# 2235854410/CCVPE

Measured on AMD Instinct MI355X. Metric: query images/sec (VIGOR, 512x512 sat / 320x640 grd), higher is better.
Workload: dtype f32; 1 GPU; vigor_samearea_fov360_b32; variant=vigor_ori_prior, batch_per_gpu=32, global_batch=32, parallelism=image-parallel x1, all_gather of 20 B/query results, schedule=two streams per GPU (aerial encoder + orientation decoder on the second)

## Files before the change

ccvpe_amd/csrc/ccvpe_api.hip:

```cpp
#include "ccvpe_internal.h"

namespace ccvpe { thread_local unsigned long long g_launches = 0; }
static thread_local std::string g_err_storage;
std::string& ccvpe_err() { return g_err_storage; }
int ccvpe_fail(int code, const char* fmt, ...) {
    char buf[1024];
    va_list ap;
    va_start(ap, fmt);
    vsnprintf(buf, sizeof(buf), fmt, ap);
    va_end(ap);
    g_err_storage = buf;
    return code;
}

__global__ __launch_bounds__(256) void checksum_kernel(const uint32_t* __restrict__ p, size_t n, unsigned long long* out) {
    unsigned long long s = 0;
    for (size_t i = (size_t)blockIdx.x * 256 + threadIdx.x; i < n; i += (size_t)gridDim.x * 256) s += (unsigned long long)p[i] * (unsigned long long)((i & 1023) + 1);
    for (int o = 32; o > 0; o >>= 1) s += __shfl_down(s, o);
    if ((threadIdx.x & 63) == 0) atomicAdd(out, s);
}


Switches read_switches() {
    Switches s;
    auto set = [](const char* name) { return getenv(name) != nullptr; };
    auto off = [](const char* name) { const char* e = getenv(name); return e && std::atoi(e) == 0; };
    if (const char* e = getenv("CCVPE_AUTOTUNE")) s.autotune = std::atoi(e) != 0;
    if (const char* e = getenv("CCVPE_FUSE_MBCONV")) s.fuse_mbconv = std::atoi(e);
    if (const char* e = getenv("CCVPE_FUSE_L1")) s.fuse_level1 = std::atoi(e) != 0;
    if (const char* e = getenv("CCVPE_L1_TILE")) s.l1_tile = std::atoi(e);
    if (const char* e = getenv("CCVPE_COMPOSE_L6")) s.compose_l6 = std::atoi(e);
    if (const char* e = getenv("CCVPE_WINOGRAD")) s.wino = std::atoi(e) != 0;
    if (const char* e = getenv("CCVPE_GRAPH")) s.graph_mode = std::atoi(e) != 0;
    if (const char* e = getenv("CCVPE_STREAMS")) s.two_streams = std::atoi(e) >= 2;
    if (const char* e = getenv("CCVPE_PRECISION")) s.precision = (std::string(e) == "bf16x3") ? 1 : 0;
    s.stem_dw = !off("CCVPE_STEM_DW");
    if (const char* e = getenv("CCVPE_FRONT_SPREAD")) s.front_spread = std::atoi(e);
    s.mbconv_image = !off("CCVPE_MBCONV_IMAGE");
    s.se_ticket = !off("CCVPE_SE_TICKET");
    if (const char* e = getenv("CCVPE_SE_PROLOGUE")) s.se_prologue = std::atoi(e) == 1;
    s.split_planes = !set("CCVPE_NO_SPLIT_PLANES");
    s.match_prep_early = !off("CCVPE_MATCH_PREP_EARLY");
    s.match_wide = !off("CCVPE_MATCH_WIDE");
    s.issue_interleaved = !off("CCVPE_ISSUE_ORDER");
    s.log_schedule = set("CCVPE_LOG_SCHEDULE");
    s.no_reuse = set("CCVPE_NO_REUSE");
// ... 290 lines not shown
            std::string nm = op.name;
            double issued = op.flops;
            if (const ConvTile* t = conv_tile(tile)) {
                nm += std::string("|") + t->name;
                if ((tile >> 8) == 255) nm += "_tailsplit";
                else if ((tile >> 8) > SPLIT_FUSED) nm += "_splitk" + std::to_string((tile >> 8) - SPLIT_FUSED) + "r";
                else if ((tile >> 8) > 1) nm += "_splitk" + std::to_string(tile >> 8);
                ConvParams q{};
                q.M = op.gemm_m; q.N = op.gemm_n;
                const double util = conv_tile_util(q, *t);
                const double mn_pad = util > 0 ? (double)op.gemm_m * op.gemm_n / util : 0.0;
                if (t->wino_f == 4) issued = 2.0 * mn_pad * 2.25 * ((op.conv_cin + 3) / 4 * 4);
                else if (t->wino_f == 2) issued = 2.0 * mn_pad * 4.0 * op.conv_cin;
                else issued = 2.0 * mn_pad * op.gemm_kpad * (t->family == TILE_BF16X3 ? 3.0 : 1.0);
            }
            h->prof.push_back({nm, ms, op.flops, op.bytes, issued});
        }
        (void)hipEventDestroy(e0);
        (void)hipEventDestroy(e1);
    }
    return 0;
}

static int run_forward(ccvpe_handle h, const ForwardCall& fc) {
    const PlanKey key = fc.plan_key();
    const int batch = fc.batch;
    if (!h || !fc.grd || (!fc.sat && !fc.cache) || (!fc.out && !key.pose)) return ccvpe_fail(CCVPE_EINVAL, "null argument");
    if (fc.cache && !fc.tile_index && batch > h->cfg.micro_batch) return ccvpe_fail(CCVPE_EINVAL, "cached forward needs batch <= micro_batch (%d)", h->cfg.micro_batch);
    if (fc.tile_index && fc.n_tiles > h->cfg.micro_batch)
        return ccvpe_fail(CCVPE_EINVAL, "n_tiles %d exceeds micro_batch (%d), the most ccvpe_encode_aerial writes", fc.n_tiles, h->cfg.micro_batch);
// ... 1096 lines not shown
```

ccvpe_amd/csrc/ccvpe_internal.h:

```cpp
#pragma once
#include "../../include/ccvpe.h"
#include "kernels.h"

#include <algorithm>
#include <cmath>
#include <cstdarg>
#include <cstdio>
#include <cstdlib>
#include <cstring>
#include <functional>
#include <map>
#include <memory>
#include <optional>
#include <set>
#include <string>
#include <type_traits>
#include <vector>

using namespace ccvpe;

std::string& ccvpe_err();
int ccvpe_fail(int code, const char* fmt, ...);
#define HIPCHK(expr)                                                                           \
    do {                                                                                       \
// ... 63 lines not shown
    int lo, hi; static_pad(k, s, lo, hi);
    return (n + lo + hi - k) / s + 1;
}
static int se_squeeze(int cin) { return std::max(1, (int)(cin * 0.25)); }
static int round_up(int a, int b) { return (a + b - 1) / b * b; }
static int deconv_width(const DecLevel& l, bool pad) {
    return (pad && l.skip > 0 && (l.dout * 4) % 64 != 0) ? round_up(l.dout, 16) : l.dout;
}

struct Switches {
    bool autotune = true;
    int fuse_mbconv = 1;
    bool fuse_level1 = true;
    int l1_tile = 1;
    std::optional<int> compose_l6;
    bool wino = true;
    int graph_mode = 0;
    bool two_streams = true;
    std::optional<int> precision;
    bool stem_dw = true;
    std::optional<int> front_spread;
    bool mbconv_image = true;
    bool se_ticket = true;
    bool se_prologue = false;
    bool split_planes = true;
    bool match_prep_early = true;
    bool match_wide = true;
    bool issue_interleaved = true;
    bool log_schedule = false;
    bool no_reuse = false;
// ... 60 lines not shown
    PackedConv head;
};
struct DecoderW {
    PackedConv deconv[6], conva[6], convb[5];
    float* tail_w = nullptr;
    float* l1_wt = nullptr;
    float tail_b[2] = {0.f, 0.f};
    float *l1_wc = nullptr, *l1_ws = nullptr, *l1_bc = nullptr;
    int l1_cx = 0, l1_cxp = 0, l1_c0 = 0, l1_ng = 0, l1_score = 0;
};
struct Level6W {
    float* wc = nullptr;
    float* bc = nullptr;
    PackedConv skip;
    int K = 0, Kc = 0, N = 0, Npad = 0;
};
static constexpr int LEVEL6_AUTO_MIN_BATCH = 8;
struct ccvpe_handle_s;
struct DecoderW;
int level6_shape(const ccvpe_handle_s* h, const DecoderW& d, const struct DecLevel& l, int& K, int& Kc, int& N, int& Npad);
int ensure_level6(ccvpe_handle_s* h, int wm);
void release_level6(ccvpe_handle_s* h);
int compose_level1(ccvpe_handle_s* h, DecoderW& d, const std::vector<float>& w, const std::vector<float>& b, const std::vector<float>& wa,
                   const std::vector<float>& ba, int cin, int nscore);
int pack_level1_tail(ccvpe_handle_s* h, DecoderW& d, const std::vector<float>& w2, const std::vector<float>& b2, int cout);

struct Tensor {
    int id = -1; int B = 0, H = 0, W = 0, C = 0;
    bool split = false;
    long long numel() const { return (long long)B * H * W * C; }
};

// ... 112 lines not shown

struct Op {
    std::string name;
    std::function<void(const Ctx&)> fn;
    std::vector<int> uses;
    double flops = 0, bytes = 0;
    std::shared_ptr<int> tile;
    int gemm_m = 0, gemm_n = 0, gemm_kpad = 0;
    int conv_cin = 0;
    bool bf16x3_only = false;
    bool wino_ok = false;
    bool wino4_ok = false;
    bool wino4x_ok = false;
    bool is_pw = false;
    bool proj_ok = false;
    int stream = 0;
    std::vector<int> wait_on;
    bool signal = false;
};

struct TapInfo { Tensor t; int coff; int C; };

struct Plan {
    PlanKey key;
    bool debug = false;
    std::vector<size_t> size;
    std::vector<size_t> off;
    std::vector<Op> ops;
    std::map<std::string, TapInfo> taps;
    size_t total = 0;
// ... 212 lines not shown
```

ccvpe_amd/csrc/ccvpe_plan.hip:

```cpp
#include "ccvpe_internal.h"

static int window_offset(const VariantSpec& vs, int level, int L) {
    const int C = vs.match_ch[level];
    return vs.centre ? (int)((double)C / 2 - (double)L / 2) : 0;
}
static int mod(int a, int m) { int r = a % m; return r < 0 ? r + m : r; }

ConvParams conv_params(const PackedConv& pc, const float* in, int in_ld, int B, int H, int W, int OH, int OW,
                              int stride, int pad_t, int pad_l, int act) {
    ConvParams p{};
    p.in = in; p.in_ld = in_ld; p.B = B; p.H = H; p.W = W; p.Cin = pc.cinp; p.OH = OH; p.OW = OW;
    p.KH = pc.KH; p.KW = pc.KW; p.stride = stride; p.pad_t = pad_t; p.pad_l = pad_l;
    p.wpk = pc.w; p.w_hi = pc.w_hi; p.w_lo = pc.w_lo; p.Kpad = pc.Kpad; p.Npad = round_up(pc.N, conv_igemm_npad()); p.nchunks = pc.nchunks; p.bias = pc.bias; p.N = pc.N; p.act = act;
    p.gate = nullptr; p.resid = nullptr; p.resid_ld = 0; p.ndst = 0; p.mode = MODE_CONV; p.deconv_cout = 0;
    p.M = B * OH * OW;
    p.in_bytes = (unsigned)((size_t)B * H * W * in_ld * sizeof(float));
    p.gate_bytes = (unsigned)((size_t)B * pc.cinp * sizeof(float));
    p.w_plane_bytes = (unsigned)((size_t)p.Npad * pc.Kpad * sizeof(unsigned short));
    p.wino_w = pc.wino; p.wino_n16 = pc.wino_n16; p.wino_bytes = (unsigned)pc.wino_bytes;
    p.wino4_w = pc.wino4; p.wino4_bytes = (unsigned)pc.wino4_bytes;
    p.wino4x_w = pc.wino4x; p.wino4x_bytes = (unsigned)pc.wino4x_bytes; p.wino4x_cfg = pc.wino4x_cfg;
    p.proj_w = pc.proj; p.proj_bytes = (unsigned)pc.proj_bytes;
    return p;
}
// ... 339 lines not shown
                : (B >= LEVEL6_AUTO_MIN_BATCH && !h->l6_failed) ? 4 : 0;
    Level6Params l6p[2] = {};
    if (l6_wm) {
        bool ok = true;
        for (int d = 0; d < 2; ++d) {
            Level6Params& q = l6p[d];
            q.wm = l6_wm; q.B = B;
            ok = ok && level6_shape(h, d ? h->ori : h->loc, d ? vs.ori[0] : vs.loc[0], q.K, q.Kc, q.N, q.Npad) == 0;
            q.R = level6_rows(B, l6_wm, &q.bm);
            ok = ok && level6_supported(q) && q.K == (d ? rpad + D : loc_in[0].C);
        }
        if (!ok && l6_forced) return ccvpe_fail(CCVPE_ESTATE, "composed level 6: the packed weights do not fit the plan's level-6 inputs");
        if (!ok) l6_wm = 0;
    }
    pl.l6_wm = l6_wm;
    Tensor skip15;
    ori_in6 = pl.alloc(B, 8, 8, rpad + D);
    pl.taps["ori_in6"] = {ori_in6, 0, ori_in6.C};

    EncOut genc, senc;
    if (!grd_cached) plan_encoder(h, pl, h->grd_enc, true, B, gh, gw, h->cfg.circular_padding != 0, nullptr, genc, "grd");
    TapDst td[5];
    for (int t = 0; t < 5; ++t) {
        td[t].n = 2;
        td[t].t[0] = loc_cat[t]; td[t].coff[0] = deconv_width(vs.loc[t], h->sw.pad_concat);
        td[t].t[1] = ori_cat[t]; td[t].coff[1] = deconv_width(vs.ori[t], h->sw.pad_concat);
    }
    if (l6_wm) td[0].n = 0;
    size_t coff[6];
    cache_layout(vs, B, coff);
// ... 68 lines not shown

    auto plan_level = [&](const DecoderW& dw, const DecLevel* lv, int j, Tensor din, Tensor cat, const std::string& tag) -> Tensor {
        const int hin = 8 << j, hout = hin * 2;
        const DecLevel& l = lv[j];
        Tensor mid = pl.alloc(B, hout, hout, l.mid);
        if (j == 0 && l6_wm) {
            const Level6W* w6 = &h->l6[&dw == &h->ori ? 1 : 0];
            const Level6Params lp = l6p[&dw == &h->ori ? 1 : 0];
            const int G = 4 * level6_positions(l6_wm);
            Tensor V = pl.alloc(G, 1, lp.R, lp.Kc), Mp = pl.alloc(G, 1, lp.R, lp.N), sk = pl.alloc(B, hout, hout, l.mid);
            const Tensor s15 = skip15;
            pl.add(tag + ".l6_transform", {din, V}, [=](const Ctx& c) {
                Level6Params q = lp; q.x = c.ptr(din); q.v = c.ptr(V);
                launch_level6_transform(q, c.stream);
            }, 0.0, 4.0 * ((double)din.numel() + (double)V.numel()));
            pl.add(tag + ".l6_gemm", {V, Mp}, [=](const Ctx& c) {
                Level6Params q = lp; q.v = c.ptr(V); q.wc = w6->wc; q.mp = c.ptr(Mp);
                launch_level6_gemm(q, c.stream);
            }, 2.0 * G * lp.R * (double)lp.N * lp.Kc, 4.0 * ((double)V.numel() + (double)G * lp.Npad * lp.Kc + (double)Mp.numel()));
            {
                const PackedConv* pc = &w6->skip;
                pl.add_conv(tag + ".conv_skip", {s15, sk}, B * hout * hout, lp.N, round_up(9 * l.skip, 32), [=](const Ctx& c, int tile) {
                    ConvParams p = conv_params(*pc, c.ptr(s15), s15.C, B, hout, hout, hout, hout, 1, 1, 1, ACT_NONE);
                    p.dst[0] = c.dst(sk); p.ndst = 1;
                    c.launch_conv(p, tile);
                }, 2.0 * B * hout * hout * 9.0 * s15.C * l.mid, 4.0 * B * hout * hout * ((double)s15.C + l.mid));
                pl.ops.back().conv_cin = s15.C;
                pl.ops.back().wino_ok = l.skip % 8 == 0;
                pl.ops.back().wino4_ok = pl.ops.back().wino_ok && lp.N >= h->sw.wino4_min_n && !h->sw.no_wino4;
                pl.ops.back().wino4x_ok = pl.ops.back().wino_ok && lp.N >= 24 && conv_wino4x_config(lp.N) >= 0 && !h->sw.no_wino4x;
            }
            pl.add(tag + ".l6_combine", {Mp, sk, mid}, [=](const Ctx& c) {
                Level6Params q = lp; q.mp = c.ptr(Mp); q.skip = c.ptr(sk); q.bc = w6->bc; q.out = c.ptr(mid);
                launch_level6_combine(q, c.stream);
            }, 0.0, 4.0 * ((double)Mp.numel() + 2.0 * (double)mid.numel()));
// ... 16 lines not shown
                pl.add_conv(tag + ".conv_a", {cat, mid}, B * hout * hout, pc->N, pc->Kpad, [=](const Ctx& c, int tile) {
                    ConvParams p = conv_params(*pc, c.ptr(cat), cat.C, B, hout, hout, hout, hout, 1, 1, 1, ACT_RELU);
                    p.in_split = cat.split; p.in_plane_bytes = (unsigned)(cat.numel() * 2);
                    p.dst[0] = c.dst(mid); p.ndst = 1;
                    c.launch_conv(p, tile);
                }, 2.0 * B * hout * hout * 9.0 * cat.C * l.mid, 4.0 * B * hout * hout * ((double)cat.C + l.mid));
                pl.ops.back().bf16x3_only = cat.split;
                pl.ops.back().conv_cin = cat.C;
                pl.ops.back().wino_ok = pc->wino != nullptr && !cat.split && h->sw.wino && h->cfg.reserved[0] == 0;
                pl.ops.back().wino4_ok = pl.ops.back().wino_ok && pc->wino4 != nullptr;
                pl.ops.back().wino4x_ok = pl.ops.back().wino_ok && pc->wino4x != nullptr;
            }
        }
        if (j == 5) return mid;
        Tensor o = pl.alloc(B, hout, hout, l.out);
        {
            const PackedConv* pc = &dw.convb[j];
            pl.add_conv(tag + ".conv_b", {mid, o}, B * hout * hout, pc->N, pc->Kpad, [=](const Ctx& c, int tile) {
                ConvParams p = conv_params(*pc, c.ptr(mid), mid.C, B, hout, hout, hout, hout, 1, 1, 1, ACT_NONE);
                p.in_split = mid.split; p.in_plane_bytes = (unsigned)(mid.numel() * 2);
                p.dst[0] = {c.ptr(o), o.C, 0}; p.ndst = 1;
                c.launch_conv(p, tile);
            }, 2.0 * B * hout * hout * 9.0 * l.mid * l.out, 4.0 * B * hout * hout * ((double)l.mid + l.out));
            pl.ops.back().bf16x3_only = mid.split;
            pl.ops.back().conv_cin = mid.C;
            pl.ops.back().wino_ok = pc->wino != nullptr && !mid.split && h->sw.wino && h->cfg.reserved[0] == 0;
            pl.ops.back().wino4_ok = pl.ops.back().wino_ok && pc->wino4 != nullptr;
            pl.ops.back().wino4x_ok = pl.ops.back().wino_ok && pc->wino4x != nullptr;
        }
        return o;
    };
// ... 323 lines not shown
```

ccvpe_amd/csrc/ccvpe_weights.hip:

```cpp
#include "ccvpe_internal.h"

#include <unistd.h>

static void add_bn(std::map<std::string, std::vector<int64_t>>& m, const std::string& p, int c) {
    m[p + ".weight"] = {c}; m[p + ".bias"] = {c}; m[p + ".running_mean"] = {c}; m[p + ".running_var"] = {c};
    m[p + ".num_batches_tracked"] = {};
}
static void add_encoder(std::map<std::string, std::vector<int64_t>>& m, const std::string& p) {
    m[p + "._conv_stem.weight"] = {32, 3, 3, 3};
    add_bn(m, p + "._bn0", 32);
    for (int i = 0; i < 16; ++i) {
        const BlockSpec& b = B0[i];
        std::string q = p + "._blocks." + std::to_string(i);
        int mid = b.cin * b.e;
        if (b.e != 1) { m[q + "._expand_conv.weight"] = {mid, b.cin, 1, 1}; add_bn(m, q + "._bn0", mid); }
        m[q + "._depthwise_conv.weight"] = {mid, 1, b.k, b.k};
        add_bn(m, q + "._bn1", mid);
        int sq = se_squeeze(b.cin);
        m[q + "._se_reduce.weight"] = {sq, mid, 1, 1}; m[q + "._se_reduce.bias"] = {sq};
        m[q + "._se_expand.weight"] = {mid, sq, 1, 1}; m[q + "._se_expand.bias"] = {mid};
        m[q + "._project_conv.weight"] = {b.cout, mid, 1, 1};
        add_bn(m, q + "._bn2", b.cout);
    }
    m[p + "._conv_head.weight"] = {1280, 320, 1, 1};
// ... 350 lines not shown
            for (int n = 0; n < N; ++n) {
                double acc = ba[n];
                for (int ky = 0; ky < 3; ++ky)
                    for (int kx = 0; kx < 3; ++kx) {
                        if ((rcase == 1 && ky == 0) || (rcase == 2 && ky == 2) || (ccase == 1 && kx == 0) || (ccase == 2 && kx == 2)) continue;
                        acc += tapsum[(size_t)(ky * 3 + kx) * N + n];
                    }
                bc[(size_t)(rcase * 3 + ccase) * N + n] = (float)acc;
            }
    {
        Level6AllocScope scope(h);
        if (int rc = upload(h, bc, &o.bc)) return rc;
        if (int rc = pack_conv(h, o.skip, N, 9, l.skip, l.skip, identity_map(l.skip), [&](int n, int t, int c) { return wa(n, t, cw + c); },
                               std::vector<float>(N, 0.f), 3, 3)) return rc;
    }
    const int P = level6_positions(wm);
    const size_t wc_bytes = (size_t)4 * P * o.Npad * o.Kc * sizeof(float), w2_bytes = (size_t)16 * N * o.Kc * sizeof(double);
    void *wc = nullptr, *w2 = nullptr;
    HIPCHK(hipMalloc(&wc, wc_bytes));
    h->l6_allocs.push_back(wc);
    o.wc = (float*)wc;
    HIPCHK(hipMemset(wc, 0, wc_bytes));
    HIPCHK(hipMalloc(&w2, w2_bytes));
    Level6ComposeParams cp{};
    cp.wm = wm; cp.dw = dc.w; cp.cw = cw; cp.dout = l.dout; cp.dkpad = dc.Kpad; cp.aw = ac.w; cp.cinw = cinw; cp.akpad = ac.Kpad;
    cp.K = o.K; cp.Kc = o.Kc; cp.N = N; cp.Npad = o.Npad; cp.w2 = (double*)w2; cp.wc = o.wc;
    launch_level6_compose(cp, nullptr);
    const hipError_t e = hipDeviceSynchronize();
    (void)hipFree(w2);
    if (e != hipSuccess) return ccvpe_fail(CCVPE_EHIP, "composing level 6 failed: %s", hipGetErrorString(e));
// ... 228 lines not shown
```

ccvpe_amd/csrc/kernels.h:

```cpp
#pragma once
#include <functional>
#include <vector>
#include <hip/hip_runtime.h>
#include <stdint.h>
#include "ticket.h"

namespace ccvpe {

extern thread_local unsigned long long g_launches;
#define CCVPE_LAUNCH(...) do { ++::ccvpe::g_launches; hipLaunchKernelGGL(__VA_ARGS__); } while (0)

struct LdsAttr { size_t set[16] = {0}; };
inline void ensure_dynamic_lds(LdsAttr& state, const void* kernel, size_t bytes) {
    int dev = 0;
    if (hipGetDevice(&dev) != hipSuccess || dev < 0 || dev >= 16) dev = 0;
    if (bytes > state.set[dev] && hipFuncSetAttribute(kernel, hipFuncAttributeMaxDynamicSharedMemorySize, (int)bytes) == hipSuccess) state.set[dev] = bytes;
}

enum Act { ACT_NONE = 0, ACT_RELU = 1, ACT_SWISH = 2 };

struct Dst {
    float* ptr;
    int ld;
    int coff;
// ... 268 lines not shown
void launch_level1_topk(const Level1Params& p, const int* index, int k, float* rows, hipStream_t s);

struct Level6Params {
    int wm;
    int B;
    int K, Kc;
    int N, Npad;
    int R, bm;
    const float* x;
    float* v;
    const float* wc;
    float* mp;
    const float* skip;
    const float* bc;
    float* out;
};
int level6_positions(int wm);
int level6_rows(int B, int wm, int* bm_out);
bool level6_supported(const Level6Params& p);
void launch_level6_transform(const Level6Params& p, hipStream_t s);
void launch_level6_gemm(const Level6Params& p, hipStream_t s);
void launch_level6_combine(const Level6Params& p, hipStream_t s);
struct Level6ComposeParams {
    int wm;
    const float* dw;
    int cw, dout, dkpad;
    const float* aw;
    int cinw, akpad;
    int K, Kc, N, Npad;
    double* w2;
    float* wc;
};
void launch_level6_compose(const Level6ComposeParams& p, hipStream_t s);

__device__ __forceinline__ float pose_angle_deg(float cs, float sn) {
    float ang = acosf(fminf(fmaxf(cs, -1.f), 1.f)) * 57.29577951308232f;
    if (sn < 0.f) { ang = fmodf(-ang, 360.f); if (ang < 0.f) ang += 360.f; }
// ... 205 lines not shown
```

ccvpe_amd/csrc/kernels_level6.hip:

```cpp
#include "igemm_common.h"

namespace ccvpe {

template <int M> struct Wino;
template <> struct Wino<4> {
    static constexpr int NP = 5;
    static __host__ __device__ constexpr float bt(int u, int i) {
        constexpr float t[5][5] = {{2, -1, -2, 1, 0}, {0, -2, -1, 1, 0}, {0, 2, -3, 1, 0}, {0, -1, 0, 1, 0}, {0, 2, -1, -2, 1}};
        return t[u][i];
    }
    static __host__ __device__ constexpr float at(int i, int u) {
        constexpr float t[4][5] = {{1, 1, 1, 1, 0}, {0, 1, -1, 2, 0}, {0, 1, 1, 4, 0}, {0, 1, -1, 8, 1}};
        return t[i][u];
    }
    static __host__ __device__ constexpr double g(int u, int a) {
        constexpr double t[5][2] = {{0.5, 0.0}, {-0.5, -0.5}, {-1.0 / 6.0, 1.0 / 6.0}, {1.0 / 6.0, 1.0 / 3.0}, {0.0, 1.0}};
        return t[u][a];
    }
};
template <> struct Wino<2> {
    static constexpr int NP = 3;
    static __host__ __device__ constexpr float bt(int u, int i) {
        constexpr float t[3][3] = {{-1, 1, 0}, {0, 1, 0}, {0, -1, 1}};
        return t[u][i];
// ... 65 lines not shown

template <int BM, int WGM, int WGN>
__global__ __launch_bounds__(256) void level6_gemm_kernel(const Level6Params p) {
    constexpr int BN = 128, MT = 32;
    constexpr int WM = BM / WGM, WN = BN / WGN, TM = WM / MT, TN = WN / MT;
    static_assert(WGM * WGN == 4 && TM >= 1 && TN >= 1 && TM * MT * WGM == BM && TN * MT * WGN == BN, "whole MFMA tiles, 4 waves");
    constexpr int AR = BM / 32, BR = BN / 32;
    constexpr int KSTEP = 8, NKK = BK / KSTEP;

    extern __shared__ __attribute__((aligned(16))) float smem[];
    float* As = smem;
    float* Bs = smem + 2 * BM * LDK;

    const int tid = threadIdx.x, lane = tid & 63, wave = tid >> 6;
    const int wm = wave / WGN, wn = wave % WGN;
    const int nbn = p.Npad / BN, mblocks = p.R / BM;
    const int lid = xcd_remap(blockIdx.x, gridDim.x);
    const int nb = lid % nbn, rest = lid / nbn;
    const int mb = rest % mblocks, g = rest / mblocks;
    const int m0 = mb * BM, n0 = nb * BN;
    const int kq = tid & 7, r0 = tid >> 3;

    const float* arow = p.v + ((size_t)g * p.R + m0 + r0) * p.Kc + kq * 4;
    const float* brow = p.wc + ((size_t)g * p.Npad + n0 + r0) * p.Kc + kq * 4;
    const size_t rstep = (size_t)32 * p.Kc;

    f32x4 ra[AR], rb[BR];
    f32x16 acc[TM][TN];
#pragma unroll
    for (int i = 0; i < TM; ++i)
#pragma unroll
        for (int j = 0; j < TN; ++j)
#pragma unroll
            for (int r = 0; r < 16; ++r) acc[i][j][r] = 0.f;

    const int nkt = p.Kc / BK;
#pragma unroll
    for (int j = 0; j < AR; ++j) ra[j] = *reinterpret_cast<const f32x4*>(arow + j * rstep);
#pragma unroll
    for (int j = 0; j < BR; ++j) rb[j] = *reinterpret_cast<const f32x4*>(brow + j * rstep);
#pragma unroll
    for (int j = 0; j < AR; ++j) *reinterpret_cast<f32x4*>(As + (r0 + 32 * j) * LDK + kq * 4) = ra[j];
#pragma unroll
    for (int j = 0; j < BR; ++j) *reinterpret_cast<f32x4*>(Bs + (r0 + 32 * j) * LDK + kq * 4) = rb[j];
    __syncthreads();

    const int a_row = wm * WM + (lane & 31);
    const int b_row = wn * WN + (lane & 31);
    const int k_lane = (lane >> 5) * 4;

    for (int kt = 0; kt < nkt; ++kt) {
// ... 48 lines not shown
#pragma unroll
            for (int i = 0; i < TM; ++i) {
                const int ml = wm * WM + i * MT + (lane & 31);
                f32x4 v;
#pragma unroll
                for (int e = 0; e < 4; ++e) v[e] = acc[i][j][4 * q + e];
                *reinterpret_cast<f32x4*>(Cs + ml * LDC + nl) = v;
            }
        }
    __syncthreads();
    constexpr int C4 = BN / 4;
    for (int it = tid; it < BM * C4; it += 256) {
        const int ml = it / C4, c4 = it - ml * C4;
        const int n = n0 + c4 * 4;
        if (n >= p.N) continue;
        *reinterpret_cast<f32x4*>(p.mp + ((size_t)g * p.R + m0 + ml) * p.N + n) = *reinterpret_cast<const f32x4*>(Cs + ml * LDC + c4 * 4);
    }
}

template <int M>
__global__ __launch_bounds__(64) void level6_combine_kernel(const Level6Params p) {
    using W = Wino<M>;
    constexpr int NP = W::NP, T = 8 / M;
    const int n = (blockIdx.x * 64 + threadIdx.x) * 4;
    if (n >= p.N) return;
    const int row = blockIdx.y, cls = blockIdx.z;
    const int b = row / (T * T), t = row - b * (T * T);
    const int ty = t / T, tx = t - ty * T, py = cls >> 1, px = cls & 1;
    const float* src = p.mp + ((size_t)cls * NP * NP * p.R + row) * p.N + n;
    const size_t gstride = (size_t)p.R * p.N;
    f32x4 m[NP][NP];
// ... 19 lines not shown
            f32x4 s = {0.f, 0.f, 0.f, 0.f};
#pragma unroll
            for (int v = 0; v < NP; ++v)
                if (W::at(j, v) != 0.f) s += W::at(j, v) * c[i][v];
            const int oy = 2 * (M * ty + i) + py, ox = 2 * (M * tx + j) + px;
            const int rcase = oy == 0 ? 1 : oy == 15 ? 2 : 0, ccase = ox == 0 ? 1 : ox == 15 ? 2 : 0;
            const size_t e = ((size_t)(b * 16 + oy) * 16 + ox) * p.N + n;
            s += *reinterpret_cast<const f32x4*>(p.skip + e);
            s += *reinterpret_cast<const f32x4*>(p.bc + (rcase * 3 + ccase) * p.N + n);
#pragma unroll
            for (int q = 0; q < 4; ++q) s[q] = fmaxf(s[q], 0.f);
            *reinterpret_cast<f32x4*>(p.out + e) = s;
        }
}

bool level6_supported(const Level6Params& p) {
    int bm = 0;
    return (p.wm == 4 || p.wm == 2) && p.B > 0 && p.K > 0 && p.K % 4 == 0 && p.Kc % BK == 0 && p.Kc >= p.K && p.N > 0 && p.N % 4 == 0 &&
           p.Npad % 128 == 0 && p.Npad >= p.N && p.R == level6_rows(p.B, p.wm, &bm) && p.bm == bm;
}

void launch_level6_transform(const Level6Params& p, hipStream_t s) {
    const dim3 grid((p.Kc / 4 + 127) / 128, p.R, 4);
    if (p.wm == 4) CCVPE_LAUNCH(level6_transform_kernel<4>, grid, dim3(128), 0, s, p);
    else CCVPE_LAUNCH(level6_transform_kernel<2>, grid, dim3(128), 0, s, p);
}

template <int BM, int WGM, int WGN>
static void launch_gemm_t(const Level6Params& p, hipStream_t s) {
    constexpr size_t lds = std::max<size_t>(2 * (BM + 128) * LDK, BM * (128 + 4)) * sizeof(float);
    static LdsAttr attr;
    auto kern = level6_gemm_kernel<BM, WGM, WGN>;
    ensure_dynamic_lds(attr, reinterpret_cast<const void*>(kern), lds);
    const int blocks = 4 * level6_positions(p.wm) * (p.R / BM) * (p.Npad / 128);
    CCVPE_LAUNCH(kern, dim3(blocks), dim3(256), lds, s, p);
}
void launch_level6_gemm(const Level6Params& p, hipStream_t s) {
    if (p.bm == 128) launch_gemm_t<128, 2, 2>(p, s);
    else if (p.bm == 64) launch_gemm_t<64, 2, 2>(p, s);
    else launch_gemm_t<32, 1, 4>(p, s);
}

void launch_level6_combine(const Level6Params& p, hipStream_t s) {
    const int t = 8 / p.wm;
    const dim3 grid((p.N / 4 + 63) / 64, p.B * t * t, 4);
    if (p.wm == 4) CCVPE_LAUNCH(level6_combine_kernel<4>, grid, dim3(64), 0, s, p);
    else CCVPE_LAUNCH(level6_combine_kernel<2>, grid, dim3(64), 0, s, p);
}

__device__ __forceinline__ int k_index_dev(int cin, int taps, int tap, int c) {
    const int full = cin / 32, cg = c / 32;
    const int g = cg < full ? cg * 4 * taps + tap * 4 + (c % 32) / 8 : full * 4 * taps + tap * ((cin % 32) / 8) + (c - full * 32) / 8;
    return g * 8 + (c % 8);
}

// ... 89 lines not shown
```

Before: 2740 queries/s.

## Run level-6 3x3 skip and conv_b as Winograd F(4,3) grouped GEMMs

Replaces the implicit-GEMM conv_skip and conv_b 3x3 convolutions at decoder level 6 (16x16 maps) with Winograd F(4x4,3x3): input-transform, 36 batched GEMMs, and inverse-transform kernels, using pre-packed transformed weights. When the tile sizes match, the skip-conv GEMM is merged into the existing level-6 deconvolution GEMM launch as a second segment with XCD-aware block remapping. This cuts the multiply count and launch count at batch >= 16, but adds transform kernels, extra scratch buffers, and fp32 Winograd rounding error.

New measurement: 2762 queries/s (median of 6 runs). No clear change (+0.8%).

```diff
diff --git a/ccvpe_amd/csrc/ccvpe_api.hip b/ccvpe_amd/csrc/ccvpe_api.hip
--- a/ccvpe_amd/csrc/ccvpe_api.hip
+++ b/ccvpe_amd/csrc/ccvpe_api.hip
@@ -30,6 +30,7 @@
     if (const char* e = getenv("CCVPE_FUSE_L1")) s.fuse_level1 = std::atoi(e) != 0;
     if (const char* e = getenv("CCVPE_L1_TILE")) s.l1_tile = std::atoi(e);
     if (const char* e = getenv("CCVPE_COMPOSE_L6")) s.compose_l6 = std::atoi(e);
+    if (const char* e = getenv("CCVPE_L6_GEMM")) s.l6_gemm = std::atoi(e);
     if (const char* e = getenv("CCVPE_WINOGRAD")) s.wino = std::atoi(e) != 0;
     if (const char* e = getenv("CCVPE_GRAPH")) s.graph_mode = std::atoi(e) != 0;
     if (const char* e = getenv("CCVPE_STREAMS")) s.two_streams = std::atoi(e) >= 2;
@@ -350,6 +351,7 @@
                 else if (t->wino_f == 2) issued = 2.0 * mn_pad * 4.0 * op.conv_cin;
                 else issued = 2.0 * mn_pad * op.gemm_kpad * (t->family == TILE_BF16X3 ? 3.0 : 1.0);
             }
+            else if (!op.form.empty()) nm += "|" + op.form;
             h->prof.push_back({nm, ms, op.flops, op.bytes, issued});
         }
         (void)hipEventDestroy(e0);
diff --git a/ccvpe_amd/csrc/ccvpe_internal.h b/ccvpe_amd/csrc/ccvpe_internal.h
--- a/ccvpe_amd/csrc/ccvpe_internal.h
+++ b/ccvpe_amd/csrc/ccvpe_internal.h
@@ -101,6 +101,7 @@
     bool fuse_level1 = true;
     int l1_tile = 1;
     std::optional<int> compose_l6;
+    std::optional<int> l6_gemm;
     bool wino = true;
     int graph_mode = 0;
     bool two_streams = true;
@@ -191,8 +192,13 @@
     float* bc = nullptr;
     PackedConv skip;
     int K = 0, Kc = 0, N = 0, Npad = 0;
+    float* w3skip = nullptr;
+    float* w3b = nullptr;
+    int K3s = 0, Kc3s = 0, K3b = 0, Kc3b = 0, N3b = 0, Npad3b = 0;
 };
 static constexpr int LEVEL6_AUTO_MIN_BATCH = 8;
+static constexpr int LEVEL6_GEMM_AUTO_MIN_BATCH = 16;
+static_assert(LEVEL6_GEMM_AUTO_MIN_BATCH >= 10, "batches below 10 keep conv_skip / conv_b");
 struct ccvpe_handle_s;
 struct DecoderW;
 int level6_shape(const ccvpe_handle_s* h, const DecoderW& d, const struct DecLevel& l, int& K, int& Kc, int& N, int& Npad);
@@ -335,6 +341,7 @@
     bool wino4x_ok = false;
     bool is_pw = false;
     bool proj_ok = false;
+    std::string form;
     int stream = 0;
     std::vector<int> wait_on;
     bool signal = false;
diff --git a/ccvpe_amd/csrc/ccvpe_plan.hip b/ccvpe_amd/csrc/ccvpe_plan.hip
--- a/ccvpe_amd/csrc/ccvpe_plan.hip
+++ b/ccvpe_amd/csrc/ccvpe_plan.hip
@@ -377,6 +377,20 @@
         if (!ok) l6_wm = 0;
     }
     pl.l6_wm = l6_wm;
+    bool l6_gemm = l6_wm == 4 && (h->sw.l6_gemm ? *h->sw.l6_gemm == 1 : B >= LEVEL6_GEMM_AUTO_MIN_BATCH);
+    for (int d = 0; d < 2 && l6_gemm; ++d) {
+        const DecoderW& dw = d ? h->ori : h->loc;
+        const DecLevel& l = d ? vs.ori[0] : vs.loc[0];
+        const PackedConv& cb = dw.convb[0];
+        Level6Conv3Params sk3{}, b3{};
+        sk3.B = b3.B = B;
+        sk3.K = l.skip; sk3.Kc = round_up(l.skip, 32); sk3.N = l6p[d].N; sk3.Npad = l6p[d].Npad; sk3.R = level6_rows3(B, l6p[d].bm, &sk3.bm);
+        b3.K = l.mid; b3.Kc = round_up(l.mid, 32); b3.N = l.out; b3.Npad = round_up(l.out, 128); b3.R = level6_rows3(B, 0, &b3.bm);
+        const bool ok = cb.w && cb.cinp == l.mid && cb.N == l.out && l6p[d].N == l.mid && TAP_C[0] == l.skip && level6_conv3_supported(sk3) &&
+                        level6_conv3_supported(b3);
+        if (!ok && h->sw.l6_gemm) return ccvpe_fail(CCVPE_ESTATE, "CCVPE_L6_GEMM=1: the level-6 3x3 layers do not fit the grouped GEMM");
+        if (!ok) l6_gemm = false;
+    }
     Tensor skip15;
     ori_in6 = pl.alloc(B, 8, 8, rpad + D);
     pl.taps["ori_in6"] = {ori_in6, 0, ori_in6.C};
@@ -475,11 +489,49 @@
                 Level6Params q = lp; q.x = c.ptr(din); q.v = c.ptr(V);
                 launch_level6_transform(q, c.stream);
             }, 0.0, 4.0 * ((double)din.numel() + (double)V.numel()));
-            pl.add(tag + ".l6_gemm", {V, Mp}, [=](const Ctx& c) {
-                Level6Params q = lp; q.v = c.ptr(V); q.wc = w6->wc; q.mp = c.ptr(Mp);
-                launch_level6_gemm(q, c.stream);
-            }, 2.0 * G * lp.R * (double)lp.N * lp.Kc, 4.0 * ((double)V.numel() + (double)G * lp.Npad * lp.Kc + (double)Mp.numel()));
-            {
+            if (l6_gemm) {
+                Level6Conv3Params sp{};
+                sp.B = B; sp.K = s15.C; sp.Kc = round_up(s15.C, 32); sp.N = lp.N; sp.Npad = lp.Npad;
+                sp.R = level6_rows3(B, lp.bm, &sp.bm);
+                Tensor V3 = pl.alloc(36, 1, sp.R, sp.Kc), Mp3 = pl.alloc(36, 1, sp.R, sp.N);
+                const bool one_launch = sp.bm == lp.bm;
+                pl.add(tag + ".l6_transform3", {s15, V3}, [=](const Ctx& c) {
+                    Level6Conv3Params q = sp; q.x = c.ptr(s15); q.v = c.ptr(V3);
+                    launch_level6_transform3(q, c.stream);
+                }, 0.0, 4.0 * ((double)s15.numel() + (double)V3.numel()));
+                const double flop1 = 2.0 * G * lp.R * (double)lp.N * lp.Kc, flop3 = 2.0 * 36 * sp.R * (double)sp.N * sp.Kc;
+                const double byte1 = 4.0 * ((double)V.numel() + (double)G * lp.Npad * lp.Kc + (double)Mp.numel());
+                const double byte3 = 4.0 * ((double)V3.numel() + 36.0 * sp.Npad * sp.Kc + (double)Mp3.numel());
+                if (one_launch) {
+                    pl.add(tag + ".l6_gemm_s", {V, V3, Mp, Mp3}, [=](const Ctx& c) {
+                        Level6Params q = lp;
+                        Level6Conv3Params q3 = sp; q3.v = c.ptr(V3); q3.w = w6->w3skip; q3.mp = c.ptr(Mp3);
+                        q.nseg = 2;
+                        q.seg[0] = {0, G, lp.R, lp.Kc, c.ptr(V), w6->wc, c.ptr(Mp)};
+                        q.seg[1] = level6_conv3_segment(q3);
+                        launch_level6_gemm(q, c.stream);
+                    }, flop1 + flop3, byte1 + byte3);
+                    pl.ops.back().form = "l6_wino4_" + std::to_string(sp.bm) + "x128";
+                } else {
+                    pl.add(tag + ".l6_gemm", {V, Mp}, [=](const Ctx& c) {
+                        Level6Params q = lp; q.v = c.ptr(V); q.wc = w6->wc; q.mp = c.ptr(Mp);
+                        launch_level6_gemm(q, c.stream);
+                    }, flop1, byte1);
+                    pl.add(tag + ".l6_gemm3", {V3, Mp3}, [=](const Ctx& c) {
+                        Level6Conv3Params q = sp; q.v = c.ptr(V3); q.w = w6->w3skip; q.mp = c.ptr(Mp3);
+                        launch_level6_gemm3(q, c.stream);
+                    }, flop3, byte3);
+                    pl.ops.back().form = "l6_wino4_" + std::to_string(sp.bm) + "x128";
+                }
+                pl.add(tag + ".l6_inverse3", {Mp3, sk}, [=](const Ctx& c) {
+                    Level6Conv3Params q = sp; q.mp = c.ptr(Mp3); q.out = c.ptr(sk);
+                    launch_level6_inverse3(q, c.stream);
+                }, 0.0, 4.0 * ((double)Mp3.numel() + (double)sk.numel()));
+            } else {
+                pl.add(tag + ".l6_gemm", {V, Mp}, [=](const Ctx& c) {
+                    Level6Params q = lp; q.v = c.ptr(V); q.wc = w6->wc; q.mp = c.ptr(Mp);
+                    launch_level6_gemm(q, c.stream);
+                }, 2.0 * G * lp.R * (double)lp.N * lp.Kc, 4.0 * ((double)V.numel() + (double)G * lp.Npad * lp.Kc + (double)Mp.numel()));
                 const PackedConv* pc = &w6->skip;
                 pl.add_conv(tag + ".conv_skip", {s15, sk}, B * hout * hout, lp.N, round_up(9 * l.skip, 32), [=](const Ctx& c, int tile) {
                     ConvParams p = conv_params(*pc, c.ptr(s15), s15.C, B, hout, hout, hout, hout, 1, 1, 1, ACT_NONE);
@@ -526,7 +578,27 @@
         }
         if (j == 5) return mid;
         Tensor o = pl.alloc(B, hout, hout, l.out);
-        {
+        if (j == 0 && l6_gemm) {
+            const Level6W* w6 = &h->l6[&dw == &h->ori ? 1 : 0];
+            const float* bias = dw.convb[0].bias;
+            Level6Conv3Params bp{};
+            bp.B = B; bp.K = mid.C; bp.Kc = round_up(mid.C, 32); bp.N = l.out; bp.Npad = round_up(l.out, 128);
+            bp.R = level6_rows3(B, 0, &bp.bm);
+            Tensor V3 = pl.alloc(36, 1, bp.R, bp.Kc), Mp3 = pl.alloc(36, 1, bp.R, bp.N);
+            pl.add(tag + ".l6_transform3b", {mid, V3}, [=](const Ctx& c) {
+                Level6Conv3Params q = bp; q.x = c.ptr(mid); q.v = c.ptr(V3);
+                launch_level6_transform3(q, c.stream);
+            }, 0.0, 4.0 * ((double)mid.numel() + (double)V3.numel()));
+            pl.add(tag + ".l6_gemm3b", {V3, Mp3}, [=](const Ctx& c) {
+                Level6Conv3Params q = bp; q.v = c.ptr(V3); q.w = w6->w3b; q.mp = c.ptr(Mp3);
+                launch_level6_gemm3(q, c.stream);
+            }, 2.0 * 36 * bp.R * (double)bp.N * bp.Kc, 4.0 * ((double)V3.numel() + 36.0 * bp.Npad * bp.Kc + (double)Mp3.numel()));
+            pl.ops.back().form = "l6_wino4_" + std::to_string(bp.bm) + "x128";
+            pl.add(tag + ".l6_inverse3b", {Mp3, o}, [=](const Ctx& c) {
+                Level6Conv3Params q = bp; q.mp = c.ptr(Mp3); q.bias = bias; q.out = c.ptr(o);
+                launch_level6_inverse3(q, c.stream);
+            }, 0.0, 4.0 * ((double)Mp3.numel() + (double)o.numel()));
+        } else {
             const PackedConv* pc = &dw.convb[j];
             pl.add_conv(tag + ".conv_b", {mid, o}, B * hout * hout, pc->N, pc->Kpad, [=](const Ctx& c, int tile) {
                 ConvParams p = conv_params(*pc, c.ptr(mid), mid.C, B, hout, hout, hout, hout, 1, 1, 1, ACT_NONE);
diff --git a/ccvpe_amd/csrc/ccvpe_weights.hip b/ccvpe_amd/csrc/ccvpe_weights.hip
--- a/ccvpe_amd/csrc/ccvpe_weights.hip
+++ b/ccvpe_amd/csrc/ccvpe_weights.hip
@@ -388,6 +388,21 @@
         if (int rc = pack_conv(h, o.skip, N, 9, l.skip, l.skip, identity_map(l.skip), [&](int n, int t, int c) { return wa(n, t, cw + c); },
                                std::vector<float>(N, 0.f), 3, 3)) return rc;
     }
+    if (wm == 4 && !(h->sw.l6_gemm && *h->sw.l6_gemm == 0)) {
+        const PackedConv& bc2 = d.convb[0];
+        if (!bc2.w || bc2.cinp != l.mid || bc2.N % 4 || l.mid % 4) return ccvpe_fail(CCVPE_ESTATE, "conv6.2 cannot run as groups of the level-6 GEMM");
+        std::vector<float> bw((size_t)round_up(bc2.N, conv_igemm_npad()) * bc2.Kpad);
+        HIPCHK(hipMemcpy(bw.data(), bc2.w, bw.size() * sizeof(float), hipMemcpyDeviceToHost));
+        o.K3s = l.skip; o.Kc3s = round_up(l.skip, 32);
+        o.K3b = l.mid; o.Kc3b = round_up(l.mid, 32); o.N3b = bc2.N; o.Npad3b = round_up(bc2.N, 128);
+        std::vector<float> w3;
+        Level6AllocScope scope(h);
+        level6_conv3_pack(N, o.Npad, o.K3s, o.Kc3s, [&](int n, int t, int c) { return wa(n, t, cw + c); }, w3);
+        if (int rc = upload(h, w3, &o.w3skip)) return rc;
+        level6_conv3_pack(o.N3b, o.Npad3b, o.K3b, o.Kc3b,
+                          [&](int n, int t, int c) { return bw[(size_t)n * bc2.Kpad + conv_igemm_k_index(l.mid, 9, t, c)]; }, w3);
+        if (int rc = upload(h, w3, &o.w3b)) return rc;
+    }
     const int P = level6_positions(wm);
     const size_t wc_bytes = (size_t)4 * P * o.Npad * o.Kc * sizeof(float), w2_bytes = (size_t)16 * N * o.Kc * sizeof(double);
     void *wc = nullptr, *w2 = nullptr;
diff --git a/ccvpe_amd/csrc/kernels.h b/ccvpe_amd/csrc/kernels.h
--- a/ccvpe_amd/csrc/kernels.h
+++ b/ccvpe_amd/csrc/kernels.h
@@ -306,6 +306,15 @@
     const float* skip;
     const float* bc;
     float* out;
+    struct Seg {
+        int b0, ng;
+        int R, Kc;
+        const float* v;
+        const float* wc;
+        float* mp;
+    };
+    int nseg;
+    Seg seg[2];
 };
 int level6_positions(int wm);
 int level6_rows(int B, int wm, int* bm_out);
@@ -313,6 +322,26 @@
 void launch_level6_transform(const Level6Params& p, hipStream_t s);
 void launch_level6_gemm(const Level6Params& p, hipStream_t s);
 void launch_level6_combine(const Level6Params& p, hipStream_t s);
+
+struct Level6Conv3Params {
+    int B;
+    int K, Kc;
+    int N, Npad;
+    int R, bm;
+    const float* x;
+    float* v;
+    const float* w;
+    float* mp;
+    const float* bias;
+    float* out;
+};
+int level6_rows3(int B, int min_bm, int* bm_out);
+bool level6_conv3_supported(const Level6Conv3Params& p);
+void launch_level6_transform3(const Level6Conv3Params& p, hipStream_t s);
+void launch_level6_gemm3(const Level6Conv3Params& p, hipStream_t s);
+void launch_level6_inverse3(const Level6Conv3Params& p, hipStream_t s);
+Level6Params::Seg level6_conv3_segment(const Level6Conv3Params& p);
+void level6_conv3_pack(int N, int Npad, int K, int Kc, const std::function<float(int, int, int)>& get, std::vector<float>& out);
 struct Level6ComposeParams {
     int wm;
     const float* dw;
diff --git a/ccvpe_amd/csrc/kernels_level6.hip b/ccvpe_amd/csrc/kernels_level6.hip
--- a/ccvpe_amd/csrc/kernels_level6.hip
+++ b/ccvpe_amd/csrc/kernels_level6.hip
@@ -103,16 +103,25 @@
 
     const int tid = threadIdx.x, lane = tid & 63, wave = tid >> 6;
     const int wm = wave / WGN, wn = wave % WGN;
-    const int nbn = p.Npad / BN, mblocks = p.R / BM;
-    const int lid = xcd_remap(blockIdx.x, gridDim.x);
+    const int xcd = blockIdx.x & 7, idx = blockIdx.x >> 3;
+    const int nb0 = p.nseg > 1 ? p.seg[1].b0 : (int)gridDim.x;
+    const int q0 = nb0 >> 3, r0x = nb0 & 7, n0x = q0 + (xcd < r0x ? 1 : 0);
+    const bool second = idx >= n0x;
+    const int lid = !second ? xcd * q0 + min(xcd, r0x) + idx
+                            : xcd * (((int)gridDim.x >> 3) - q0) + min(xcd, (int)gridDim.x & 7) - min(xcd, r0x) + (idx - n0x);
+    const int R = second ? p.seg[1].R : p.seg[0].R, Kc = second ? p.seg[1].Kc : p.seg[0].Kc;
+    const float* sv = second ? p.seg[1].v : p.seg[0].v;
+    const float* sw = second ? p.seg[1].wc : p.seg[0].wc;
+    float* smp = second ? p.seg[1].mp : p.seg[0].mp;
+    const int nbn = p.Npad / BN, mblocks = R / BM;
     const int nb = lid % nbn, rest = lid / nbn;
     const int mb = rest % mblocks, g = rest / mblocks;
     const int m0 = mb * BM, n0 = nb * BN;
     const int kq = tid & 7, r0 = tid >> 3;
 
-    const float* arow = p.v + ((size_t)g * p.R + m0 + r0) * p.Kc + kq * 4;
-    const float* brow = p.wc + ((size_t)g * p.Npad + n0 + r0) * p.Kc + kq * 4;
-    const size_t rstep = (size_t)32 * p.Kc;
+    const float* arow = sv + ((size_t)g * R + m0 + r0) * Kc + kq * 4;
+    const float* brow = sw + ((size_t)g * p.Npad + n0 + r0) * Kc + kq * 4;
+    const size_t rstep = (size_t)32 * Kc;
 
     f32x4 ra[AR], rb[BR];
     f32x16 acc[TM][TN];
@@ -123,7 +132,7 @@
 #pragma unroll
             for (int r = 0; r < 16; ++r) acc[i][j][r] = 0.f;
 
-    const int nkt = p.Kc / BK;
+    const int nkt = Kc / BK;
 #pragma unroll
     for (int j = 0; j < AR; ++j) ra[j] = *reinterpret_cast<const f32x4*>(arow + j * rstep);
 #pragma unroll
@@ -202,7 +211,7 @@
         const int ml = it / C4, c4 = it - ml * C4;
         const int n = n0 + c4 * 4;
         if (n >= p.N) continue;
-        *reinterpret_cast<f32x4*>(p.mp + ((size_t)g * p.R + m0 + ml) * p.N + n) = *reinterpret_cast<const f32x4*>(Cs + ml * LDC + c4 * 4);
+        *reinterpret_cast<f32x4*>(smp + ((size_t)g * R + m0 + ml) * p.N + n) = *reinterpret_cast<const f32x4*>(Cs + ml * LDC + c4 * 4);
     }
 }
 
@@ -252,6 +261,145 @@
         }
 }
 
+__device__ __forceinline__ f32x4 fma4(float a, f32x4 x, f32x4 y) {
+    return f32x4{fmaf(a, x.x, y.x), fmaf(a, x.y, y.y), fmaf(a, x.z, y.z), fmaf(a, x.w, y.w)};
+}
+__device__ __forceinline__ void w4_bt4(const f32x4* d, f32x4* t) {
+    const f32x4 a = fma4(-4.f, d[2], d[4]), b = fma4(-4.f, d[1], d[3]);
+    const f32x4 c = d[4] - d[2], e = d[3] - d[1];
+    t[0] = fma4(4.f, d[0], fma4(-5.f, d[2], d[4]));
+    t[1] = a + b;
+    t[2] = a - b;
+    t[3] = fma4(2.f, e, c);
+    t[4] = fma4(-2.f, e, c);
+    t[5] = fma4(4.f, d[1], fma4(-5.f, d[3], d[5]));
+}
+__device__ __forceinline__ void w4_at4(const f32x4* m, f32x4* y) {
+    const f32x4 s1 = m[1] + m[2], d1 = m[1] - m[2], s2 = m[3] + m[4], d2 = m[3] - m[4];
+    y[0] = m[0] + s1 + s2;
+    y[1] = fma4(2.f, d2, d1);
+    y[2] = fma4(4.f, s2, s1);
+    y[3] = fma4(8.f, d2, d1) + m[5];
+}
+
+int level6_rows3(int B, int min_bm, int* bm_out) {
+    const int rows = B * 16;
+    const int bm = std::max(min_bm, rows > 32 ? 64 : 32);
+    if (bm_out) *bm_out = bm;
+    return (rows + bm - 1) / bm * bm;
+}
+
+__global__ __launch_bounds__(128) void level6_transform3_kernel(const Level6Conv3Params p) {
+    const int k = (blockIdx.x * 128 + threadIdx.x) * 4;
+    if (k >= p.Kc) return;
+    const int row = blockIdx.y;
+    const int b = row >> 4, t = row & 15;
+    const int y0 = 4 * (t >> 2) - 1, x0 = 4 * (t & 3) - 1;
+    const bool live = b < p.B && k < p.K;
+    f32x4 c[6][6];
+#pragma unroll
+    for (int i = 0; i < 6; ++i) {
+        f32x4 d[6];
+#pragma unroll
+        for (int j = 0; j < 6; ++j) {
+            const int y = y0 + i, x = x0 + j;
+            d[j] = f32x4{0.f, 0.f, 0.f, 0.f};
+            if (live && (unsigned)y < 16u && (unsigned)x < 16u) d[j] = *reinterpret_cast<const f32x4*>(p.x + ((size_t)(b * 16 + y) * 16 + x) * p.K + k);
+        }
+        w4_bt4(d, c[i]);
+    }
+    float* dst = p.v + (size_t)row * p.Kc + k;
+    const size_t gstride = (size_t)p.R * p.Kc;
+#pragma unroll
+    for (int v = 0; v < 6; ++v) {
+        f32x4 in[6], o[6];
+#pragma unroll
+        for (int i = 0; i < 6; ++i) in[i] = c[i][v];
+        w4_bt4(in, o);
+#pragma unroll
+        for (int u = 0; u < 6; ++u) {
+            *reinterpret_cast<f32x4*>(dst + (size_t)(u * 6 + v) * gstride) = o[u];
+            __builtin_amdgcn_sched_barrier(0);
+            asm volatile("s_nop 1");
+            __builtin_amdgcn_sched_barrier(0);
+        }
+    }
+}
+
+__global__ __launch_bounds__(64) void level6_inverse3_kernel(const Level6Conv3Params p) {
+    const int n = (blockIdx.x * 64 + threadIdx.x) * 4;
+    if (n >= p.N) return;
+    const int row = blockIdx.y;
+    const int b = row >> 4, t = row & 15;
+    const float* src = p.mp + (size_t)row * p.N + n;
+    const size_t gstride = (size_t)p.R * p.N;
+    f32x4 c[6][4];
+#pragma unroll
+    for (int u = 0; u < 6; ++u) {
+        f32x4 m[6];
+#pragma unroll
+        for (int v = 0; v < 6; ++v) m[v] = *reinterpret_cast<const f32x4*>(src + (size_t)(u * 6 + v) * gstride);
+        w4_at4(m, c[u]);
+    }
+    f32x4 bias = {0.f, 0.f, 0.f, 0.f};
+    if (p.bias) bias = *reinterpret_cast<const f32x4*>(p.bias + n);
+    float* dst = p.out + ((size_t)(b * 16 + 4 * (t >> 2)) * 16 + 4 * (t & 3)) * p.N + n;
+#pragma unroll
+    for (int j = 0; j < 4; ++j) {
+        f32x4 in[6], y[4];
+#pragma unroll
+        for (int u = 0; u < 6; ++u) in[u] = c[u][j];
+        w4_at4(in, y);
+#pragma unroll
+        for (int i = 0; i < 4; ++i) {
+            *reinterpret_cast<f32x4*>(dst + (size_t)(i * 16 + j) * p.N) = y[i] + bias;
+            __builtin_amdgcn_sched_barrier(0);
+            asm volatile("s_nop 1");
+            __builtin_amdgcn_sched_barrier(0);
+        }
+    }
+}
+
+bool level6_conv3_supported(const Level6Conv3Params& p) {
+    return p.B > 0 && p.K > 0 && p.K % 4 == 0 && p.Kc % BK == 0 && p.Kc >= p.K && p.N > 0 && p.N % 4 == 0 && p.Npad % 128 == 0 &&
+           p.Npad >= p.N && (p.bm == 32 || p.bm == 64 || p.bm == 128) && p.R % p.bm == 0 && p.R >= 16 * p.B;
+}
+
+void launch_level6_transform3(const Level6Conv3Params& p, hipStream_t s) {
+    CCVPE_LAUNCH(level6_transform3_kernel, dim3((p.Kc / 4 + 127) / 128, p.R), dim3(128), 0, s, p);
+}
+
+void launch_level6_inverse3(const Level6Conv3Params& p, hipStream_t s) {
+    CCVPE_LAUNCH(level6_inverse3_kernel, dim3((p.N / 4 + 63) / 64, p.B * 16), dim3(64), 0, s, p);
+}
+
+Level6Params::Seg level6_conv3_segment(const Level6Conv3Params& p) { return {0, 36, p.R, p.Kc, p.v, p.w, p.mp}; }
+
+void launch_level6_gemm3(const Level6Conv3Params& p, hipStream_t s) {
+    Level6Params q{};
+    q.N = p.N; q.Npad = p.Npad; q.bm = p.bm;
+    q.nseg = 1;
+    q.seg[0] = level6_conv3_segment(p);
+    launch_level6_gemm(q, s);
+}
+
+void level6_conv3_pack(int N, int Npad, int K, int Kc, const std::function<float(int, int, int)>& get, std::vector<float>& out) {
+    static const double G[6][3] = {{0.25, 0.0, 0.0}, {-1.0 / 6, -1.0 / 6, -1.0 / 6}, {-1.0 / 6, 1.0 / 6, -1.0 / 6},
+                                   {1.0 / 24, 1.0 / 12, 1.0 / 6}, {1.0 / 24, -1.0 / 12, 1.0 / 6}, {0.0, 0.0, 1.0}};
+    out.assign((size_t)36 * Npad * Kc, 0.f);
+    for (int n = 0; n < N; ++n)
+        for (int c = 0; c < K; ++c) {
+            double g[3][3], tmp[6][3];
+            for (int i = 0; i < 3; ++i)
+                for (int j = 0; j < 3; ++j) g[i][j] = (double)get(n, i * 3 + j, c);
+            for (int r = 0; r < 6; ++r)
+                for (int j = 0; j < 3; ++j) tmp[r][j] = G[r][0] * g[0][j] + G[r][1] * g[1][j] + G[r][2] * g[2][j];
+            for (int r = 0; r < 6; ++r)
+                for (int q = 0; q < 6; ++q)
+                    out[((size_t)(r * 6 + q) * Npad + n) * Kc + c] = (float)(tmp[r][0] * G[q][0] + tmp[r][1] * G[q][1] + tmp[r][2] * G[q][2]);
+        }
+}
+
 bool level6_supported(const Level6Params& p) {
     int bm = 0;
     return (p.wm == 4 || p.wm == 2) && p.B > 0 && p.K > 0 && p.K % 4 == 0 && p.Kc % BK == 0 && p.Kc >= p.K && p.N > 0 && p.N % 4 == 0 &&
@@ -270,13 +418,23 @@
     static LdsAttr attr;
     auto kern = level6_gemm_kernel<BM, WGM, WGN>;
     ensure_dynamic_lds(attr, reinterpret_cast<const void*>(kern), lds);
-    const int blocks = 4 * level6_positions(p.wm) * (p.R / BM) * (p.Npad / 128);
-    CCVPE_LAUNCH(kern, dim3(blocks), dim3(256), lds, s, p);
+    int blocks = 0;
+    Level6Params q = p;
+    for (int i = 0; i < q.nseg; ++i) {
+        q.seg[i].b0 = blocks;
+        blocks += q.seg[i].ng * (q.seg[i].R / BM) * (q.Npad / 128);
+    }
+    CCVPE_LAUNCH(kern, dim3(blocks), dim3(256), lds, s, q);
 }
 void launch_level6_gemm(const Level6Params& p, hipStream_t s) {
-    if (p.bm == 128) launch_gemm_t<128, 2, 2>(p, s);
-    else if (p.bm == 64) launch_gemm_t<64, 2, 2>(p, s);
-    else launch_gemm_t<32, 1, 4>(p, s);
+    Level6Params q = p;
+    if (q.nseg == 0) {
+        q.nseg = 1;
+        q.seg[0] = {0, 4 * level6_positions(p.wm), p.R, p.Kc, p.v, p.wc, p.mp};
+    }
+    if (q.bm == 128) launch_gemm_t<128, 2, 2>(q, s);
+    else if (q.bm == 64) launch_gemm_t<64, 2, 2>(q, s);
+    else launch_gemm_t<32, 1, 4>(q, s);
 }
 
 void launch_level6_combine(const Level6Params& p, hipStream_t s) {
```
